# OpenPPL/ppl.llm.serving

Hardware: AMD Instinct MI355X
Metric: decode tokens/sec, LLaMA-7B int8 (W8A16), max-running-batch 1024 (higher is better)
Workload: dtype fp16 activations, int8 weights (W8A16), int8-g8 KV, fp32 accumulate

## Files before the change

ppl.llm.serving_amd/csrc/k_common.h:

```cpp
#pragma once
#include <hip/hip_runtime.h>
#include <hip/hip_fp16.h>
#include <stdint.h>
#include <stdlib.h>

namespace pplhip {

typedef _Float16 h8 __attribute__((ext_vector_type(8)));
typedef _Float16 h4 __attribute__((ext_vector_type(4)));
typedef _Float16 h2 __attribute__((ext_vector_type(2)));
typedef float f4 __attribute__((ext_vector_type(4)));

constexpr int WAVE = 64;

inline int tune_int(const char* name, int dflt) {
#ifdef PPLHIP_TUNING_BUILD
    const char* v = getenv(name);
    return v ? atoi(v) : dflt;
#else
    (void)name;
    return dflt;
#endif
}
inline bool tune_set(const char* name) {
// ... 105 lines not shown
    return w;
}
__device__ __forceinline__ h8 cvt_i4x8_f16(uint32_t w) {
    const uint32_t lo = w & 0x0f0f0f0fu, hi = (w >> 4) & 0x0f0f0f0fu;
    const uint32_t b0 = __builtin_amdgcn_perm(hi, lo, 0x05010400u), b1 = __builtin_amdgcn_perm(hi, lo, 0x07030602u);
    const h2 bias = {(_Float16)1032.0f, (_Float16)1032.0f};
    const h2 a = __builtin_bit_cast(h2, __builtin_amdgcn_perm(0x64646464u, b0, 0x04010400u)) - bias;
    const h2 b = __builtin_bit_cast(h2, __builtin_amdgcn_perm(0x64646464u, b0, 0x04030402u)) - bias;
    const h2 c = __builtin_bit_cast(h2, __builtin_amdgcn_perm(0x64646464u, b1, 0x04010400u)) - bias;
    const h2 d = __builtin_bit_cast(h2, __builtin_amdgcn_perm(0x64646464u, b1, 0x04030402u)) - bias;
    return h8{a[0], a[1], b[0], b[1], c[0], c[1], d[0], d[1]};
}
__device__ __forceinline__ h8 cvt_i4x8_f16(uint32_t w, _Float16 s) { return cvt_i4x8_f16(w) * s; }

#ifndef PPLHIP_KV_NT
#define PPLHIP_KV_NT 1
#endif
typedef uint32_t kv_u32x4 __attribute__((ext_vector_type(4)));
__device__ __forceinline__ uint4 kv_stream_load(const uint4* p) {
#if PPLHIP_KV_NT
    return __builtin_bit_cast(uint4, __builtin_nontemporal_load(reinterpret_cast<const kv_u32x4*>(p)));
#else
    return *p;
#endif
}
__device__ __forceinline__ uint32_t kv_stream_load(const uint32_t* p) {
#if PPLHIP_KV_NT
    return __builtin_nontemporal_load(p);
#else
    return *p;
#endif
}

struct KvStrides {
    int64_t sL, sKV, sH, sN;
};
__host__ __device__ inline KvStrides kv_strides(int layout, int64_t N, int64_t L, int64_t h, int64_t d) {
    KvStrides s;
    switch (layout) {
        case 0: s.sN = L * 2 * h * d; s.sL = 2 * h * d; s.sKV = h * d; s.sH = d; break;
        case 1: s.sL = N * 2 * h * d; s.sN = 2 * h * d; s.sKV = h * d; s.sH = d; break;
        case 2: s.sL = 2 * N * h * d; s.sKV = N * h * d; s.sN = h * d; s.sH = d; break;
        default: s.sL = 2 * h * N * d; s.sKV = h * N * d; s.sH = N * d; s.sN = d; break;
    }
    return s;
}

struct KvAddr {
    void* cache;
    uint16_t* scale;
    int64_t sKV, sH, sN;
    int64_t ssKV, ssH, ssN;
    int32_t mode, page_size;
    int32_t page_shift;
};

__device__ __forceinline__ int64_t kv_slot(const KvAddr& a, const int64_t* __restrict__ cache_indices, int64_t max_pages,
                                           int64_t b, int64_t pos) {
    if (a.mode == 0) return cache_indices[b] + pos;
    if (a.page_shift >= 0) {
        const int64_t pg = pos >> a.page_shift;
        return (cache_indices[b * max_pages + pg] << a.page_shift) + (pos & (int64_t)(a.page_size - 1));
    }
    const int64_t pg = pos / a.page_size;
    return cache_indices[b * max_pages + pg] * a.page_size + (pos - pg * a.page_size);
}
// ... 3 lines not shown
```

ppl.llm.serving_amd/csrc/k_elem.hip:

```cpp
#include <stdlib.h>
#include "kernels.h"

namespace pplhip {

__global__ __launch_bounds__(256) void embedding_kernel(const int64_t* __restrict__ ids, const uint4* __restrict__ table,
                                                        int chunks , uint4* __restrict__ out) {
    const int64_t t = blockIdx.x;
    const int64_t row = ids[t];
    for (int c = threadIdx.x; c < chunks; c += 256) out[t * chunks + c] = table[row * chunks + c];
}

hipError_t launch_embedding(hipStream_t s, const int64_t* token_ids, const uint16_t* table, int64_t T, int hidden,
                            uint16_t* out) {
    if (T == 0) return hipSuccess;
    hipLaunchKernelGGL(embedding_kernel, dim3((unsigned)T), dim3(256), 0, s, token_ids, (const uint4*)table, hidden / 8,
                       (uint4*)out);
    return hipGetLastError();
}

__global__ __launch_bounds__(256) void gather_last_rows_kernel(const int64_t* __restrict__ seq_starts, const uint4* __restrict__ x, int chunks,
                                                               uint4* __restrict__ out) {
    const int64_t r = blockIdx.x, src = seq_starts[r + 1] - 1;
    for (int c = threadIdx.x; c < chunks; c += 256) out[r * chunks + c] = x[src * chunks + c];
}

hipError_t launch_gather_last_rows(hipStream_t s, const uint16_t* x, const int64_t* seq_starts, int64_t B, int hidden, uint16_t* out) {
    if (B == 0) return hipSuccess;
    if (hidden % 8) return hipErrorInvalidValue;
    hipLaunchKernelGGL(gather_last_rows_kernel, dim3((unsigned)B), dim3(256), 0, s, seq_starts, (const uint4*)x, hidden / 8, (uint4*)out);
    return hipGetLastError();
}

template <int MAXC, int NT = 256, bool F8 = false>
__global__ __launch_bounds__(NT) void rmsnorm_kernel(const uint4* x , const uint4* __restrict__ skip,
                                                      const uint4* __restrict__ w, float eps, int chunks, int hidden,
                                                      const int64_t* __restrict__ gather, uint4* __restrict__ out,
                                                      uint4* residual_out, int8_t* __restrict__ qout, float* __restrict__ sx, SplitSlabs sl) {
    __shared__ float red[NT / 64];
    __shared__ float redq[NT / 64];
    const int64_t r = blockIdx.x;
    const int64_t src = gather ? gather[r + 1] - 1 : r;
    float v[MAXC][8];
    float ss = 0.f;
#pragma unroll
    for (int i = 0; i < MAXC; ++i) {
        const int c = threadIdx.x + i * NT;
        if (c < chunks) {
            unpack8(x[src * chunks + c], v[i]);
            if (skip || sl.splits) {
                float sk[8];
                if (sl.splits) slab_load8(sl, src, c * 8, sk);
                else unpack8(skip[src * chunks + c], sk);
#pragma unroll
                for (int j = 0; j < 8; ++j) v[i][j] = round_h(v[i][j] + sk[j]);
                if (residual_out) residual_out[r * chunks + c] = pack8(v[i]);
            } else if (residual_out) {
                residual_out[r * chunks + c] = pack8(v[i]);
            }
#pragma unroll
            for (int j = 0; j < 8; ++j) ss += v[i][j] * v[i][j];
        }
    }
    uint4 wraw[MAXC];
#pragma unroll
    for (int i = 0; i < MAXC; ++i) {
        const int c = threadIdx.x + i * NT;
        wraw[i] = c < chunks ? w[c] : make_uint4(0, 0, 0, 0);
    }
    ss = wave_sum(ss);
    if ((threadIdx.x & 63) == 0) red[threadIdx.x >> 6] = ss;
    __syncthreads();
    ss = red[0] + red[1] + red[2] + red[3];
#pragma unroll
    for (int wv = 4; wv < NT / 64; ++wv) ss += red[wv];
    const float inv = 1.0f / sqrtf(ss / (float)hidden + eps);
    if (!qout) {
#pragma unroll
        for (int i = 0; i < MAXC; ++i) {
            const int c = threadIdx.x + i * NT;
            if (c < chunks) {
                float wf[8], o[8];
                unpack8(wraw[i], wf);
#pragma unroll
                for (int j = 0; j < 8; ++j) o[j] = v[i][j] * inv * wf[j];
                out[r * chunks + c] = pack8(o);
            }
        }
        return;
    }
    float amax = 0.f;
#pragma unroll
    for (int i = 0; i < MAXC; ++i) {
        const int c = threadIdx.x + i * NT;
        if (c < chunks) {
            float wf[8];
            unpack8(wraw[i], wf);
#pragma unroll
            for (int j = 0; j < 8; ++j) {
                v[i][j] = round_h(v[i][j] * inv * wf[j]);
                amax = fmaxf(amax, fabsf(v[i][j]));
            }
        }
    }
#pragma unroll
    for (int o = 32; o > 0; o >>= 1) amax = fmaxf(amax, __shfl_xor(amax, o));
    if ((threadIdx.x & 63) == 0) redq[threadIdx.x >> 6] = amax;
    __syncthreads();
    amax = fmaxf(fmaxf(redq[0], redq[1]), fmaxf(redq[2], redq[3]));
#pragma unroll
    for (int wv = 4; wv < NT / 64; ++wv) amax = fmaxf(amax, redq[wv]);
    if constexpr (F8) {
        const int e = fp8_row_exp(amax);
        if (threadIdx.x == 0) sx[r] = pow2f(e);
#pragma unroll
        for (int i = 0; i < MAXC; ++i) {
            const int c = threadIdx.x + i * NT;
            if (c < chunks) {
                uint32_t lo = 0, hi = 0;
// ... 126 lines not shown
```

ppl.llm.serving_amd/csrc/k_gemm.hip:

```cpp
#include <stdarg.h>
#include <stdio.h>
#include <stdlib.h>

#include <algorithm>

#include <type_traits>
#include "k_gemm_dev.h"

namespace pplhip {

void LinearRoute::add(const char* fmt, ...) {
    if (!buf || cap <= 0 || len >= cap - 1) return;
    if (len > 0) buf[len++] = ' ';
    va_list ap;
    va_start(ap, fmt);
    const int n = vsnprintf(buf + len, (size_t)(cap - len), fmt, ap);
    va_end(ap);
    len = n < 0 ? len : (len + n < cap - 1 ? len + n : cap - 1);
    buf[len] = 0;
}

template <int WQ, int EPI>
__global__ __launch_bounds__(256) void gemm_kernel(const uint16_t* __restrict__ x, const void* __restrict__ wv,
                                                   const uint16_t* __restrict__ scale, int64_t M, int N, int K, int group,
// ... 129 lines not shown
        __syncthreads();
        if (t + 1 < ktiles) {
            store_tile();
            __syncthreads();
        }
    }

#pragma unroll
    for (int i = 0; i < 4; ++i) {
        const int n = n0 + wn * 64 + i * 16 + kq * 4;
        if (n >= N) continue;
        float sc[4] = {1.f, 1.f, 1.f, 1.f};
        if constexpr (WQ == 8) {
            const uint2 s2 = *reinterpret_cast<const uint2*>(scale + n);
            const h4 sh = __builtin_bit_cast(h4, s2);
#pragma unroll
            for (int r = 0; r < 4; ++r) sc[r] = (float)sh[r];
        }
#pragma unroll
        for (int j = 0; j < 4; ++j) {
            const int64_t m = m0 + wm * 64 + j * 16 + l15;
            if (m >= M) continue;
            store4<EPI>(yv, ldy, m, n, acc[i][j][0] * sc[0], acc[i][j][1] * sc[1], acc[i][j][2] * sc[2], acc[i][j][3] * sc[3]);
        }
    }
}

struct DmaKernel { int wq, epi, stages, wl, bm, maxg; };
template <int WQ, int EPI, int G_ST, int WL, int BM = G_BM, int MAXG = W4_MAXG>
__global__ __launch_bounds__(WL == 6 ? 768 : (WL == 5 ? 512 : 256)) void gemm_dma_kernel(const uint16_t* __restrict__ x, const void* __restrict__ wv,
                                                             const uint16_t* __restrict__ scale, int64_t M, int N, int K,
                                                             void* __restrict__ yv, int64_t ldy, int n_tiles, int m_tiles,
                                                             int map_mode, int kt_per_split, float* __restrict__ ws) {
    __shared__ __attribute__((aligned(16))) char smem[gemm_dma_lds_bytes<WQ, G_ST, BM, MAXG>()];
    gemm_dma_body<WQ, EPI, G_ST, WL, BM>(x, wv, scale, M, N, K, yv, ldy, n_tiles, m_tiles, map_mode, kt_per_split, ws, (int)blockIdx.x,
                                     (int)blockIdx.y, (int)gridDim.y, smem);
}

constexpr int S_KS = 2;
constexpr int S_WB = G_BN * G_BK * S_KS;
template <int BM> constexpr int s_xb() { return S_KS * BM * G_BK * 2; }
struct Half128Kernel { int epi, st, bm; };

template <int EPI, int ST, int BM>
__global__ __launch_bounds__(256) void gemm_w8_half128_kernel(const uint16_t* __restrict__ x, const int8_t* __restrict__ w,
                                                              const uint16_t* __restrict__ scale, int64_t M, int N, int K,
                                                              void* __restrict__ yv, int64_t ldy, int n_tiles, int kt_per_split,
                                                              float* __restrict__ ws) {
    constexpr int XB = s_xb<BM>(), NJ = BM / 16;
    constexpr int XP = XB / 1024, WP = S_WB / 1024, PP = (XP + WP) / 4;
    static_assert((XP + WP) % 4 == 0, "every wave issues the same number of pieces");
    extern __shared__ __attribute__((aligned(16))) char smem_h[];
    char* const Xs0 = smem_h;
    char* const Wq0 = smem_h + ST * XB;
    const int nt = blockIdx.x;
    if (nt >= n_tiles) return;
    const int n0 = nt * G_BN;
    const int split_id = blockIdx.y, n_splits = gridDim.y;
    const int tid = threadIdx.x, lane = tid & 63, wave = __builtin_amdgcn_readfirstlane(tid >> 6);
    const int l15 = lane & 15, kq = lane >> 4;
    const int nb = wave * 32;

    const char* psrc[PP];
    uint32_t pdst[PP];
    const uint32_t xbase = lds_addr(Xs0), wbase = lds_addr(Wq0);
#pragma unroll
    for (int j = 0; j < PP; ++j) {
// ... 204 lines not shown
        char* const stg = smem256;
        __syncthreads();
#pragma unroll
        for (int i = 0; i < 2; ++i) {
            const int nl = wn * 32 + i * 16 + kq * 4;
            const int nc = n0 + nl < N ? n0 + nl : 0;
            const h4 sh = __builtin_bit_cast(h4, *reinterpret_cast<const uint2*>(scale + nc));
#pragma unroll
            for (int j = 0; j < 16; ++j) {
                const float v0 = acc[i][j][0] * (float)sh[0], v1 = acc[i][j][1] * (float)sh[1], v2 = acc[i][j][2] * (float)sh[2],
                            v3 = acc[i][j][3] * (float)sh[3];
                char* dst = stg + (j * 16 + l15) * ROWB;
                if constexpr (EPI == EPI_F16) {
                    const h4 o = {to_h(v0), to_h(v1), to_h(v2), to_h(v3)};
                    *reinterpret_cast<uint2*>(dst + nl * 2) = __builtin_bit_cast(uint2, o);
                } else {
                    const float g0 = round_h(v0), u0 = round_h(v1), g1 = round_h(v2), u1 = round_h(v3);
                    const h2 o = {to_h(g0 / (1.0f + __expf(-g0)) * u0), to_h(g1 / (1.0f + __expf(-g1)) * u1)};
                    *reinterpret_cast<uint32_t*>(dst + nl) = __builtin_bit_cast(uint32_t, o);
                }
            }
        }
        __syncthreads();
        uint16_t* const y = reinterpret_cast<uint16_t*>(yv);
        const int nout = EPI == EPI_SWIGLU ? N / 2 : N, c0 = EPI == EPI_SWIGLU ? n0 / 2 : n0;
#pragma unroll 4
        for (int c = tid; c < H_BM * CPR; c += 512) {
            const int row = c / CPR, ch = c - row * CPR;
            const uint4 v = *reinterpret_cast<const uint4*>(stg + row * ROWB + ch * 16);
            const int64_t m = m0 + row;
            const int col = c0 + ch * 8;
            if (m < M) {
                if (col + 8 <= nout) {
                    *reinterpret_cast<uint4*>(y + m * ldy + col) = v;
                } else {
                    const uint16_t* e = reinterpret_cast<const uint16_t*>(&v);
                    for (int k = 0; k < 8; ++k)
                        if (col + k < nout) y[m * ldy + col + k] = e[k];
                }
            }
        }
        return;
    }
#pragma unroll
    for (int i = 0; i < 2; ++i) {
        const int n = n0 + wn * 32 + i * 16 + kq * 4;
        if (n >= N) continue;
        const h4 sh = __builtin_bit_cast(h4, *reinterpret_cast<const uint2*>(scale + n));
#pragma unroll
        for (int j = 0; j < 16; ++j) {
            const int64_t m = m0 + wm * 128 + j * 16 + l15;
            if (m >= M) continue;
            store4<EPI>(yv, ldy, m, n, acc[i][j][0] * (float)sh[0], acc[i][j][1] * (float)sh[1], acc[i][j][2] * (float)sh[2],
                        acc[i][j][3] * (float)sh[3]);
        }
    }
}

template <int WQ, int MT, int EPI, int NW>
__global__ __launch_bounds__(NW * 64) void gemv_kernel(const uint16_t* __restrict__ x, const void* __restrict__ wv,
                                                   const uint16_t* __restrict__ scale, int64_t M, int N, int K, int group,
                                                   void* __restrict__ yv, int64_t ldy) {
    constexpr int KL = WQ == 8 ? 16 : (WQ == 4 ? 32 : 8);
    constexpr int KSTEP = KL * 4;
    constexpr int NKS = KL / 8;
    __shared__ __attribute__((aligned(16))) float red[NW - 1][MT][64][4];
    const int tid = threadIdx.x, lane = tid & 63, wave = tid >> 6;
// ... 373 lines not shown
```

ppl.llm.serving_amd/csrc/k_gemm_dev.h:

```cpp
#pragma once
#include "kernels.h"
#include "k_launch.h"

namespace pplhip {

constexpr int G_BN = 128, G_BM = 128, G_BK = 64;

__device__ __forceinline__ int g_swz(int row, int chunk) { return chunk ^ ((row >> 1) & 7); }

enum { EPI_F16 = 0, EPI_F32 = 1, EPI_SWIGLU = 2 };
template <int EPI>
__device__ __forceinline__ void store4(void* yv, int64_t ldy, int64_t m, int n, float v0, float v1, float v2, float v3) {
    if constexpr (EPI == EPI_F32) {
        *reinterpret_cast<float4*>(reinterpret_cast<float*>(yv) + m * ldy + n) = make_float4(v0, v1, v2, v3);
    } else if constexpr (EPI == EPI_F16) {
        const h4 o = {to_h(v0), to_h(v1), to_h(v2), to_h(v3)};
        *reinterpret_cast<uint2*>(reinterpret_cast<uint16_t*>(yv) + m * ldy + n) = __builtin_bit_cast(uint2, o);
    } else {
        const float g0 = round_h(v0), u0 = round_h(v1), g1 = round_h(v2), u1 = round_h(v3);
        const h2 o = {to_h(g0 / (1.0f + __expf(-g0)) * u0), to_h(g1 / (1.0f + __expf(-g1)) * u1)};
        *reinterpret_cast<uint32_t*>(reinterpret_cast<uint16_t*>(yv) + m * ldy + (n >> 1)) = __builtin_bit_cast(uint32_t, o);
    }
}

template <class F>
inline void dispatch_epi(int epi, F&& f) {
    if (epi == EPI_F32) f(int_c<EPI_F32>{}); else if (epi == EPI_F16) f(int_c<EPI_F16>{}); else f(int_c<EPI_SWIGLU>{});
}
template <class F>
inline void for_each_epi(F&& f) { f(int_c<EPI_F16>{}); f(int_c<EPI_F32>{}); f(int_c<EPI_SWIGLU>{}); }

__device__ __forceinline__ int w_swz(int row) { return (0x1320 >> (((row >> 2) & 3) * 4)) & 3; }

__device__ __forceinline__ h8 cvt_i4x8_f16(uint32_t w, h2 sc) {
    const uint32_t ev = w & 0x0f0f0f0fu, od = (w >> 4) & 0x0f0f0f0fu;
    const h2 bias = {(_Float16)1032.0f, (_Float16)1032.0f};
    const h2 a = (__builtin_bit_cast(h2, __builtin_amdgcn_perm(od, ev, 0x0c040c00u) | 0x64006400u) - bias) * sc;
    const h2 b = (__builtin_bit_cast(h2, __builtin_amdgcn_perm(od, ev, 0x0c050c01u) | 0x64006400u) - bias) * sc;
    const h2 c = (__builtin_bit_cast(h2, __builtin_amdgcn_perm(od, ev, 0x0c060c02u) | 0x64006400u) - bias) * sc;
    const h2 d = (__builtin_bit_cast(h2, __builtin_amdgcn_perm(od, ev, 0x0c070c03u) | 0x64006400u) - bias) * sc;
    return h8{a[0], a[1], b[0], b[1], c[0], c[1], d[0], d[1]};
}

__device__ __forceinline__ void glds16(const void* gsrc, uint32_t lds_wave_base ) {
    uint32_t keep;
    asm volatile("s_mov_b32 %0, m0\n\ts_mov_b32 m0, %2\n\ts_nop 0\n\tglobal_load_lds_dwordx4 %1, off\n\ts_mov_b32 m0, %0"
                 : "=&s"(keep)
                 : "v"(gsrc), "s"(lds_wave_base)
                 : "memory");
}
__device__ __forceinline__ uint32_t lds_addr(const void* p) {
    return (uint32_t)(uintptr_t)(const __attribute__((address_space(3))) char*)p;
}

constexpr int W4_MAXG = 64;

template <int WQ, int G_ST, int BM = G_BM, int MAXG = W4_MAXG>
constexpr int gemm_dma_lds_bytes() {
    constexpr int WB2 = WQ == 8 ? 2 : (WQ == 4 ? 1 : 4);
    return G_ST * (BM * G_BK * 2 + G_BN * G_BK * WB2 / 2) + (WQ == 4 ? MAXG * G_BN * 2 : 0);
}

template <int WQ, int EPI, int G_ST, int WL, int BM = G_BM>
__device__ __forceinline__ void gemm_dma_body(const uint16_t* __restrict__ x, const void* __restrict__ wv,
                                              const uint16_t* __restrict__ scale, int64_t M, int N, int K, void* __restrict__ yv,
                                              int64_t ldy, int n_tiles, int m_tiles, int map_mode, int kt_per_split,
                                              float* __restrict__ ws, int block_id, int split_id, int n_splits, char* smem) {
    constexpr int WB2 = WQ == 8 ? 2 : (WQ == 4 ? 1 : 4);
    constexpr int W_STAGE = G_BN * G_BK * WB2 / 2;
    constexpr int NT = 256;
    static_assert(BM == G_BM || (BM == 64 && WL == 1), "half-height tiles: 4-wave layout only");
    constexpr int X_DMA = BM * G_BK * 2 / (NT * 16);
    constexpr int W_DMA = W_STAGE / (NT * 16);
    uint16_t* const Xs0 = reinterpret_cast<uint16_t*>(smem);
    char* const Wq0 = smem + G_ST * BM * G_BK * 2;
    uint16_t* const Sc = reinterpret_cast<uint16_t*>(smem + G_ST * (BM * G_BK * 2 + W_STAGE));
    const char* w = reinterpret_cast<const char*>(wv);

    const int id = block_id;
    const int xcd = id & 7, slot = id >> 3;
    int nt, mt;
    if ((map_mode & 0xff) == 1) {
        const int mg = m_tiles >> 3;
        mt = xcd + 8 * (slot % mg);
        nt = slot / mg;
    } else {
        const int gm = (map_mode >> 16) & 0xff, gn = (map_mode >> 24) & 0xff;
        if (gm == 0) {
            nt = xcd + 8 * (slot / m_tiles);
            mt = slot % m_tiles;
        } else {
            const int per_super = gn * gm, sm_count = m_tiles / gm;
            const int sup = slot / per_super, within = slot % per_super;
            nt = xcd + 8 * ((sup / sm_count) * gn + within / gm);
            mt = (sup % sm_count) * gm + within % gm;
        }
    }
    if (nt >= n_tiles) return;
    const int n0 = nt * G_BN;
    const int64_t m0 = (int64_t)mt * BM;

    constexpr bool PC = WL == 5 || WL == 6;
    const bool producer = PC && threadIdx.x >= (WL == 6 ? 512 : 256);
    const int tid = PC ? (threadIdx.x & 255) : threadIdx.x, lane = tid & 63, wave = tid >> 6;
    const int kh = WL == 6 ? (int)((threadIdx.x >> 8) & 1) : 0;
    const int l15 = lane & 15, kq = lane >> 4;
    constexpr int NI = WL ? 2 : 4, NJ = WL ? BM / 16 : 4;
    const int wn = WL ? wave : wave >> 1, wm = WL ? 0 : wave & 1;
    const int nb = wn * (NI * 16), mb = wm * (NJ * 16);

    const uint16_t* xsrc[X_DMA];
    const char* wsrc[W_DMA];
#pragma unroll
    for (int j = 0; j < X_DMA; ++j) {
        const int p = j * NT + tid, row = p >> 3, pos = (p & 7) ^ ((row >> 1) & 7);
        const int c = ((pos & 3) << 1) | (pos >> 2);
        int64_t m = m0 + row;
        if (m >= M) m = M - 1;
        xsrc[j] = x + m * K + c * 8;
    }
#pragma unroll
    for (int j = 0; j < W_DMA; ++j) {
        const int p = j * NT + tid;
        if constexpr (WQ == 8) {
            const int row = p >> 2, c = (p & 3) ^ w_swz(row);
            int n = n0 + row;
            if (n >= N) n = N - 1;
            wsrc[j] = w + (int64_t)n * K + c * 16;
        } else if constexpr (WQ == 4) {
            const int row = p >> 1, c = (p & 1) ^ ((row >> 3) & 1);
            int n = n0 + row;
            if (n >= N) n = N - 1;
            wsrc[j] = w + ((int64_t)n * K) / 2 + c * 16;
        } else {
            const int row = p >> 3, pos = (p & 7) ^ ((row >> 1) & 7);
            const int c = ((pos & 3) << 1) | (pos >> 2);
// ... 19 lines not shown

    constexpr int D = G_ST - 1;
    const int kt_all = K / G_BK;
    const int kt0 = split_id * kt_per_split;
    const int ktiles = (kt0 + kt_per_split < kt_all) ? kt_per_split : kt_all - kt0;
    if constexpr (WQ == 4) {
        const int G = K / 128, g0 = kt0 >> 1, ng = (ktiles + 1) >> 1;
        for (int e = tid; e < ng * G_BN; e += NT) {
            const int row = e / ng, g = e - row * ng;
            int n = n0 + row;
            if (n >= N) n = N - 1;
            Sc[g * G_BN + row] = scale[(int64_t)n * G + g0 + g];
        }
        asm volatile("s_waitcnt vmcnt(0)" ::: "memory");
    }
#pragma unroll
    for (int d = 0; d < D; ++d) {
        if (d < ktiles && (!PC || producer)) issue(d, (kt0 + d) * G_BK);
    }
    int st = 0, stn = D;
    h2 gsc[NI];
    if (PC && producer) {
        for (int t = 0; t < ktiles; ++t) {
            const int younger = (ktiles - 1 - t) < (D - 1) ? (ktiles - 1 - t) : (D - 1);
            constexpr int PT = X_DMA + W_DMA;
            if (younger >= 2) asm volatile("s_waitcnt vmcnt(%0)" ::"n"(2 * PT) : "memory");
            else if (younger == 1) asm volatile("s_waitcnt vmcnt(%0)" ::"n"(PT) : "memory");
            else asm volatile("s_waitcnt vmcnt(0)" ::: "memory");
            __syncthreads();
            if (t + D < ktiles) issue(stn, (kt0 + t + D) * G_BK);
            stn = stn == G_ST - 1 ? 0 : stn + 1;
        }
        if constexpr (WL == 6) { __syncthreads(); __syncthreads(); }
        return;
    }
    for (int t = 0; t < ktiles; ++t) {
        const int younger = (ktiles - 1 - t) < (D - 1) ? (ktiles - 1 - t) : (D - 1);
        if constexpr (!PC) {
            constexpr int PT = X_DMA + W_DMA;
            if (map_mode & 0x200) {}
            else if (younger >= 2) asm volatile("s_waitcnt vmcnt(%0)" ::"n"(2 * PT) : "memory");
            else if (younger == 1) asm volatile("s_waitcnt vmcnt(%0)" ::"n"(PT) : "memory");
            else asm volatile("s_waitcnt vmcnt(0)" ::: "memory");
        }
        __syncthreads();
        if constexpr (!PC) if (t + D < ktiles && !(map_mode & 0x100)) issue(stn, (kt0 + t + D) * G_BK);
        const uint16_t* xs = Xs0 + st * (BM * G_BK);
        const char* wq = Wq0 + st * W_STAGE;
        st = st == G_ST - 1 ? 0 : st + 1;
        stn = stn == G_ST - 1 ? 0 : stn + 1;
        uint4 wraw[NI];
        if constexpr (WQ == 8) {
#pragma unroll
            for (int i = 0; i < NI; ++i) {
                const int row = nb + i * 16 + l15;
                wraw[i] = *reinterpret_cast<const uint4*>(&wq[row * G_BK + (kq ^ w_swz(row)) * 16]);
            }
        } else if constexpr (WQ == 4) {
#pragma unroll
            for (int i = 0; i < NI; ++i) {
                const int row = nb + i * 16 + l15;
                const uint2 v = *reinterpret_cast<const uint2*>(&wq[row * 32 + ((kq ^ (((row >> 3) & 1) << 1)) * 8)]);
                wraw[i].x = v.x; wraw[i].y = v.y;
            }
            if ((t & 1) == 0) {
#pragma unroll
// ... 17 lines not shown
                    const int row = nb + i * 16 + l15;
                    a[i] = __builtin_bit_cast(h8, *reinterpret_cast<const uint4*>(&wq[(row * G_BK + g_swz(row, ks * 4 + kq) * 8) * 2]));
                }
            }
#pragma unroll
            for (int j = 0; j < NJ; ++j) {
                const int row = mb + j * 16 + l15;
                bfr[j] = __builtin_bit_cast(h8, *reinterpret_cast<const uint4*>(&xs[row * G_BK + g_swz(row, ks * 4 + kq) * 8]));
            }
#ifdef GEMM_SETPRIO
            __builtin_amdgcn_s_setprio(1);
#endif
#pragma unroll
            for (int i = 0; i < NI; ++i)
#pragma unroll
                for (int j = 0; j < NJ; ++j) acc[i][j] = __builtin_amdgcn_mfma_f32_16x16x32_f16(a[i], bfr[j], acc[i][j], 0, 0, 0);
#ifdef GEMM_SETPRIO
            __builtin_amdgcn_s_setprio(0);
#endif
        }
    }

    if constexpr (WL == 6) {
        float4* red = reinterpret_cast<float4*>(smem);
        __syncthreads();
        if (kh == 1) {
#pragma unroll
            for (int i = 0; i < NI; ++i)
#pragma unroll
                for (int j = 0; j < NJ; ++j)
                    red[((wave * NI + i) * NJ + j) * 64 + lane] = make_float4(acc[i][j][0], acc[i][j][1], acc[i][j][2], acc[i][j][3]);
        }
        __syncthreads();
        if (kh == 1) return;
#pragma unroll
        for (int i = 0; i < NI; ++i)
#pragma unroll
            for (int j = 0; j < NJ; ++j) {
                const float4 o = red[((wave * NI + i) * NJ + j) * 64 + lane];
                acc[i][j][0] += o.x; acc[i][j][1] += o.y; acc[i][j][2] += o.z; acc[i][j][3] += o.w;
            }
    }
    if (n_splits > 1) {
        float* slab = ws + (int64_t)split_id * M * N;
#pragma unroll
        for (int i = 0; i < NI; ++i) {
            const int n = n0 + nb + i * 16 + kq * 4;
            if (n >= N) continue;
#pragma unroll
            for (int j = 0; j < NJ; ++j) {
                const int64_t m = m0 + mb + j * 16 + l15;
                if (m < M) *reinterpret_cast<float4*>(slab + m * N + n) = make_float4(acc[i][j][0], acc[i][j][1], acc[i][j][2], acc[i][j][3]);
            }
        }
        return;
    }
#pragma unroll
    for (int i = 0; i < NI; ++i) {
        const int n = n0 + nb + i * 16 + kq * 4;
        if (n >= N) continue;
        h4 sh = {(_Float16)1.0f, (_Float16)1.0f, (_Float16)1.0f, (_Float16)1.0f};
        if constexpr (WQ == 8) sh = __builtin_bit_cast(h4, *reinterpret_cast<const uint2*>(scale + n));
#pragma unroll
        for (int j = 0; j < NJ; ++j) {
            const int64_t m = m0 + mb + j * 16 + l15;
            if (m >= M) continue;
            store4<EPI>(yv, ldy, m, n, acc[i][j][0] * (float)sh[0], acc[i][j][1] * (float)sh[1], acc[i][j][2] * (float)sh[2],
                        acc[i][j][3] * (float)sh[3]);
        }
    }
}


}
// ... 1 lines not shown
```

ppl.llm.serving_amd/csrc/k_gemm_wide.hip:

```cpp
#include <stdlib.h>
#include "k_gemm_dev.h"

namespace pplhip {

namespace {

constexpr int WD_BM = 128, WD_NP = 4;
constexpr int WD_XB = WD_BM * G_BK * 2;
constexpr int WD_XP = WD_XB / 1024;

template <int EPI, int ST, int NC, int ABL = 0>
__global__ __launch_bounds__((NC + WD_NP) * 64) void gemm_w8_wide_kernel(const uint16_t* __restrict__ x, const int8_t* __restrict__ w,
                                                                  const uint16_t* __restrict__ scale, int64_t M, int N, int K,
                                                                  void* __restrict__ yv, int64_t ldy, int n_tiles, int m_tiles) {
    constexpr int WD_BN = 32 * NC, WD_NC = NC;
    constexpr int WD_WB = WD_BN * G_BK, WD_WP = WD_WB / 1024;
    constexpr int WD_PP = (WD_XP + WD_WP + WD_NP - 1) / WD_NP;
    extern __shared__ __attribute__((aligned(16))) char smem_wd[];
    char* const Xs0 = smem_wd;
    char* const Wq0 = smem_wd + ST * WD_XB;

    const int id = blockIdx.x;
    const int xcd = id & 7, slot = id >> 3;
    const int nt = xcd + 8 * (slot / m_tiles);
    const int mt = slot % m_tiles;
    if (nt >= n_tiles) return;
    const int n0 = nt * WD_BN;
    const int64_t m0 = (int64_t)mt * WD_BM;

    const int tid = threadIdx.x, lane = tid & 63, wave = __builtin_amdgcn_readfirstlane(tid >> 6);
    const int ktiles = K / G_BK;
    constexpr int D = ST - 1;

    if (wave >= WD_NC) {
        const int pw = wave - WD_NC;
        const char* psrc[WD_PP];
        uint32_t pdst[WD_PP];
        const uint32_t xbase = lds_addr(Xs0), wbase = lds_addr(Wq0);
        const int npc = (WD_XP + WD_WP - pw + WD_NP - 1) / WD_NP;
#pragma unroll
        for (int j = 0; j < WD_PP; ++j) {
            const int P = pw + WD_NP * j;
            if (j < WD_XP / WD_NP) {
                const int p = P * 64 + lane, row = p >> 3, pos = (p & 7) ^ ((row >> 1) & 7);
                const int c = ((pos & 3) << 1) | (pos >> 2);
                int64_t m = m0 + row;
                if (m >= M) m = M - 1;
                psrc[j] = reinterpret_cast<const char*>(x + m * K + c * 8);
                pdst[j] = __builtin_amdgcn_readfirstlane(xbase + P * 1024);
            } else {
                const int Pw = (P < WD_XP + WD_WP ? P : WD_XP) - WD_XP;
                const int p = Pw * 64 + lane, row = p >> 2, c = (p & 3) ^ w_swz(row);
                int n = n0 + row;
                if (n >= N) n = N - 1;
                psrc[j] = reinterpret_cast<const char*>(w) + (int64_t)n * K + c * 16;
                pdst[j] = __builtin_amdgcn_readfirstlane(wbase + Pw * 1024);
            }
        }
#define WD_PRODUCE(KT, STG)                                                                                                          \
    do {                                                                                                                             \
        _Pragma("unroll") for (int j = 0; j < WD_PP; ++j)                                                                            \
            if (j < npc)                                                                                                             \
            glds16(psrc[j] + (int64_t)(KT) * (j < WD_XP / WD_NP ? G_BK * 2 : G_BK), pdst[j] + (STG) * (j < WD_XP / WD_NP ? WD_XB : WD_WB)); \
    } while (0)
#pragma unroll
        for (int d = 0; d < D; ++d)
            if (d < ktiles) WD_PRODUCE(d, d);
        int stn = D % ST;
        for (int t = 0; t < ktiles; ++t) {
            const int younger = (ktiles - 1 - t) < (D - 1) ? (ktiles - 1 - t) : (D - 1);
            if (younger >= 2) {
                if (npc == WD_PP) asm volatile("s_waitcnt vmcnt(%0)" ::"n"(2 * WD_PP) : "memory");
                else asm volatile("s_waitcnt vmcnt(%0)" ::"n"(2 * WD_PP - 2) : "memory");
            } else if (younger == 1) {
                if (npc == WD_PP) asm volatile("s_waitcnt vmcnt(%0)" ::"n"(WD_PP) : "memory");
                else asm volatile("s_waitcnt vmcnt(%0)" ::"n"(WD_PP - 1) : "memory");
            } else {
                asm volatile("s_waitcnt vmcnt(0)" ::: "memory");
            }
            if (!(ABL & 8)) __syncthreads();
            if (t + D < ktiles && !(ABL & 1)) WD_PRODUCE(t + D, stn);
            stn = stn == ST - 1 ? 0 : stn + 1;
        }
#undef WD_PRODUCE
        return;
    }

    const int l15 = lane & 15, kq = lane >> 4;
    const int nb = wave * 32;
    f4 acc[2][8];
#pragma unroll
    for (int i = 0; i < 2; ++i)
#pragma unroll
        for (int j = 0; j < 8; ++j) acc[i][j] = f4{0.f, 0.f, 0.f, 0.f};
    int st = 0;
    for (int t = 0; t < ktiles; ++t) {
        if (!(ABL & 8)) __syncthreads();
        const uint16_t* xs = reinterpret_cast<const uint16_t*>(Xs0 + st * WD_XB);
        const char* wq = Wq0 + st * WD_WB;
        st = st == ST - 1 ? 0 : st + 1;
        uint4 wraw[2];
#pragma unroll
        for (int i = 0; i < 2; ++i) {
            const int row = nb + i * 16 + l15;
            wraw[i] = *reinterpret_cast<const uint4*>(&wq[row * G_BK + (kq ^ w_swz(row)) * 16]);
        }
#pragma unroll
        for (int ks = 0; ks < 2; ++ks) {
            h8 a[2], bfr[8];
#pragma unroll
            for (int i = 0; i < 2; ++i) {
                if constexpr (ABL & 2) a[i] = __builtin_bit_cast(h8, make_uint4(wraw[i].x, wraw[i].y, wraw[i].z ^ ks, wraw[i].w));
                else a[i] = cvt_i8x8_f16(ks == 0 ? make_uint2(wraw[i].x, wraw[i].y) : make_uint2(wraw[i].z, wraw[i].w));
            }
#pragma unroll
            for (int j = 0; j < 8; ++j) {
                const int row = j * 16 + l15;
                bfr[j] = __builtin_bit_cast(h8, *reinterpret_cast<const uint4*>(&xs[((ABL & 4) ? 0 : row * G_BK) + g_swz(row, ks * 4 + kq) * 8]));
            }
#pragma unroll
            for (int i = 0; i < 2; ++i)
#pragma unroll
                for (int j = 0; j < 8; ++j) acc[i][j] = __builtin_amdgcn_mfma_f32_16x16x32_f16(a[i], bfr[j], acc[i][j], 0, 0, 0);
        }
    }

#pragma unroll
    for (int i = 0; i < 2; ++i) {
        const int n = n0 + nb + i * 16 + kq * 4;
        if (n >= N) continue;
        const h4 sh = __builtin_bit_cast(h4, *reinterpret_cast<const uint2*>(scale + n));
#pragma unroll
        for (int j = 0; j < 8; ++j) {
            const int64_t m = m0 + j * 16 + l15;
            if (m >= M) continue;
            store4<EPI>(yv, ldy, m, n, acc[i][j][0] * (float)sh[0], acc[i][j][1] * (float)sh[1], acc[i][j][2] * (float)sh[2],
                        acc[i][j][3] * (float)sh[3]);
        }
    }
}

}

int linear_w8_wide_waves(int64_t M, int N) {
    const int64_t m_tiles = (M + WD_BM - 1) / WD_BM;
    const int64_t tiles = (N + 383) / 384 * m_tiles, rounds = (tiles + 255) / 256;
    const double eff = (double)N * (double)M / ((double)rounds * 256.0 * 384.0 * WD_BM);
    return (eff >= 0.85 && (rounds <= 2 || eff >= 0.97)) ? 12 : 0;
}

hipError_t launch_linear_w8_wide(hipStream_t s, const uint16_t* x, const int8_t* w, const uint16_t* scale, int64_t M, int N, int K, void* y,
                                 int64_t ldy, int epi, int nc, LinearRoute* route) {
    if (nc != 12) return hipErrorInvalidValue;
    const int bn = 32 * nc;
    const int n_tiles = (N + bn - 1) / bn, m_tiles = (int)((M + WD_BM - 1) / WD_BM);
    constexpr int ST = 3;
    const size_t lds = (size_t)ST * (WD_XB + bn * G_BK);
    if (route) {
        route->add("kernel=gemm_w8_wide_kernel<%s,%d,%d> splits=1 reduce=none order=plain", epi_name(epi), ST, nc);
// ... 25 lines not shown
```

ppl.llm.serving_amd/csrc/k_rope_kv.hip:

```cpp
#include <stdlib.h>
#include "kernels.h"

namespace pplhip {

template <int QBIT>
__device__ __forceinline__ void store_group8(const KvAddr& kv, int kvsel, int head, int64_t slot, int ch0,
                                             const float* x ) {
    const int64_t base = (int64_t)kvsel * kv.sKV + (int64_t)head * kv.sH + slot * kv.sN + ch0;
    if constexpr (QBIT == 0) {
        *reinterpret_cast<uint4*>(reinterpret_cast<uint16_t*>(kv.cache) + base) = pack8(x);
    } else {
        float mx = 0.f;
#pragma unroll
        for (int i = 0; i < 8; ++i) mx = fmaxf(mx, fabsf(x[i]));
        const _Float16 sh = to_h(mx / 127.0f);
        const float sf = (float)sh;
        const float inv = sf > 0.f ? __fdiv_rn(1.0f, sf) : 0.f;
        uint32_t lo = 0, hi = 0;
#pragma unroll
        for (int i = 0; i < 8; ++i) {
            float q = rintf(__fmul_rn(x[i], inv));
            q = fminf(fmaxf(q, -127.f), 127.f);
            const uint32_t b = (uint32_t)(int)q & 0xffu;
            if (i < 4) lo |= b << (8 * i); else hi |= b << (8 * (i - 4));
        }
        *reinterpret_cast<uint2*>(reinterpret_cast<int8_t*>(kv.cache) + base) = make_uint2(lo, hi);
        const int64_t sbase = (int64_t)kvsel * kv.ssKV + (int64_t)head * kv.ssH + slot * kv.ssN + ch0 / 8;
        kv.scale[sbase] = __builtin_bit_cast(uint16_t, sh);
    }
}

__device__ __forceinline__ void store_fp8_row8(const KvAddr& kv, int kvsel, int head, int64_t slot, int ch0, const float* x ,
                                               int e) {
    const int64_t base = (int64_t)kvsel * kv.sKV + (int64_t)head * kv.sH + slot * kv.sN + ch0;
    const float inv = __builtin_bit_cast(float, (uint32_t)(127 - e) << 23);
    const float lim = e == 8 ? 240.0f : 448.0f;
    uint32_t lo = 0, hi = 0;
#pragma unroll
    for (int i = 0; i < 8; ++i) {
        const float y = __fmul_rn(x[i], inv);
        const uint32_t b = fp8_e4m3_rne(fminf(fmaxf(y, -lim), lim));
        if (i < 4) lo |= b << (8 * i); else hi |= b << (8 * (i - 4));
    }
    *reinterpret_cast<uint2*>(reinterpret_cast<uint8_t*>(kv.cache) + base) = make_uint2(lo, hi);
    if (ch0 == 0) kv.scale[(int64_t)kvsel * kv.ssKV + (int64_t)head * kv.ssH + slot * kv.ssN] = f2h(__builtin_bit_cast(float, (uint32_t)(127 + e) << 23));
}
__device__ __forceinline__ void store_i4_group8(const KvAddr& kv, int kvsel, int head, int64_t slot, int ch0, const float* x , float amax) {
    const float sf = kv_i4_scale(amax);
    const float inv = __fdiv_rn(1.0f, sf);
    const int64_t base = (int64_t)kvsel * kv.sKV + (int64_t)head * kv.sH + slot * kv.sN + ch0 / 2;
    *reinterpret_cast<uint32_t*>(reinterpret_cast<uint8_t*>(kv.cache) + base) = kv_i4_pack8(x, inv);
    if ((ch0 & 31) == 0) kv.scale[(int64_t)kvsel * kv.ssKV + (int64_t)head * kv.ssH + slot * kv.ssN + ch0 / 32] = f2h(sf);
}
__device__ __forceinline__ float group_max(float v, int n) {
    for (int o = 1; o < n; o <<= 1) v = fmaxf(v, __shfl_xor(v, o, 64));
    return v;
}

template <int QBIT>
__global__ __launch_bounds__(256) void rope_kv_write_kernel(uint16_t* __restrict__ qkv, const float* __restrict__ cos_sin,
                                                            KvAddr kv, const int64_t* __restrict__ seq_starts,
                                                            const int64_t* __restrict__ start_pos,
                                                            const int64_t* __restrict__ cache_indices, int64_t max_pages,
                                                            int64_t B, int64_t t0, int H, int Hkv, int D, SplitSlabs sl) {
    const int64_t t = t0 + blockIdx.x;
    int64_t b;
    {
        const int64_t g = t < B ? t : B - 1;
        int64_t lo = 0, hi = B - 1;
        if (seq_starts[g] <= t && t < seq_starts[g + 1]) {
            lo = g;
        } else {
            while (lo < hi) {
                const int64_t mid = (lo + hi + 1) >> 1;
                if (seq_starts[mid] <= t) lo = mid; else hi = mid - 1;
            }
        }
        b = lo;
    }
    const int64_t pos = start_pos[b] + (t - seq_starts[b]);
    const int64_t slot = kv_slot(kv, cache_indices, max_pages, b, pos);
    const int half = D / 2;
    const int bph = half / 8;
    const int n_rope = (H + Hkv) * bph;
    const int n_v = Hkv * (D / 8);
    const int v0 = QBIT == KV_FP8 ? (n_rope + D / 8 - 1) / (D / 8) * (D / 8) : (QBIT == KV_I4G32 ? (n_rope + 3) / 4 * 4 : n_rope);
    uint16_t* row = qkv + t * (int64_t)(H + 2 * Hkv) * D;
    const float* cs = cos_sin + pos * D;
    for (int w = blockIdx.y * 256 + threadIdx.x; w < v0 + n_v; w += 256 * gridDim.y) {
        if (w < n_rope) {
            const int head = w / bph, i0 = (w - head * bph) * 8;
            uint16_t* x = row + (int64_t)head * D;
            float a[8], bb[8], c[8], s[8], ra[8], rb[8];
            if (sl.splits) {
                slab_load8(sl, t - t0, head * D + i0, a);
                slab_load8(sl, t - t0, head * D + i0 + half, bb);
            } else {
                unpack8(*reinterpret_cast<const uint4*>(x + i0), a);
                unpack8(*reinterpret_cast<const uint4*>(x + i0 + half), bb);
            }
            *reinterpret_cast<float4*>(c) = *reinterpret_cast<const float4*>(cs + i0);
            *reinterpret_cast<float4*>(c + 4) = *reinterpret_cast<const float4*>(cs + i0 + 4);
            *reinterpret_cast<float4*>(s) = *reinterpret_cast<const float4*>(cs + half + i0);
            *reinterpret_cast<float4*>(s + 4) = *reinterpret_cast<const float4*>(cs + half + i0 + 4);
#pragma unroll
            for (int i = 0; i < 8; ++i) {
                ra[i] = round_h(__fsub_rn(__fmul_rn(a[i], c[i]), __fmul_rn(bb[i], s[i])));
                rb[i] = round_h(__fadd_rn(__fmul_rn(bb[i], c[i]), __fmul_rn(a[i], s[i])));
            }
            if (head < H) {
                *reinterpret_cast<uint4*>(x + i0) = pack8(ra);
                *reinterpret_cast<uint4*>(x + i0 + half) = pack8(rb);
            } else if constexpr (QBIT == KV_FP8) {
                float mx = 0.f;
#pragma unroll
                for (int i = 0; i < 8; ++i) mx = fmaxf(mx, fmaxf(fabsf(ra[i]), fabsf(rb[i])));
                const int e = fp8_row_exp(group_max(mx, bph));
                store_fp8_row8(kv, 0, head - H, slot, i0, ra, e);
                store_fp8_row8(kv, 0, head - H, slot, i0 + half, rb, e);
            } else if constexpr (QBIT == KV_I4G32) {
                float ma = 0.f, mb = 0.f;
#pragma unroll
                for (int i = 0; i < 8; ++i) { ma = fmaxf(ma, fabsf(ra[i])); mb = fmaxf(mb, fabsf(rb[i])); }
                if (D == 32) ma = mb = group_max(fmaxf(ma, mb), 2);
                else { ma = group_max(ma, 4); mb = group_max(mb, 4); }
                store_i4_group8(kv, 0, head - H, slot, i0, ra, ma);
                store_i4_group8(kv, 0, head - H, slot, i0 + half, rb, mb);
            } else {
                store_group8<QBIT>(kv, 0, head - H, slot, i0, ra);
                store_group8<QBIT>(kv, 0, head - H, slot, i0 + half, rb);
            }
        } else if (w >= v0) {
            const int wv = w - v0;
            const int head = wv / (D / 8), i0 = (wv - head * (D / 8)) * 8;
            float v[8];
            if (sl.splits) slab_load8(sl, t - t0, (H + Hkv + head) * D + i0, v);
            else unpack8(*reinterpret_cast<const uint4*>(row + (int64_t)(H + Hkv + head) * D + i0), v);
            if constexpr (QBIT == KV_FP8) {
                float mx = 0.f;
#pragma unroll
                for (int i = 0; i < 8; ++i) mx = fmaxf(mx, fabsf(v[i]));
                store_fp8_row8(kv, 1, head, slot, i0, v, fp8_row_exp(group_max(mx, D / 8)));
            } else if constexpr (QBIT == KV_I4G32) {
                float mx = 0.f;
#pragma unroll
// ... 44 lines not shown
```

Measured before the change: 23930.

## Stage GEMM epilogue outputs through LDS for coalesced row stores

GEMM epilogues in the wide and producer/consumer DMA kernels now write scaled fp16 or SwiGLU results into an LDS image that reuses the ring buffer. All threads then copy it out as contiguous 16-byte row chunks instead of scattered 4-element fragment stores. The aim is fully coalesced global writes of the output tile, paid for with extra barriers, LDS traffic and a larger LDS allocation for the WL6 variant. Selectable store-cache policies (write-through, nontemporal) are also added for the GEMM, norm and rope/KV stores, but they default to plain stores.

```diff
diff --git a/ppl.llm.serving_amd/csrc/k_common.h b/ppl.llm.serving_amd/csrc/k_common.h
--- a/ppl.llm.serving_amd/csrc/k_common.h
+++ b/ppl.llm.serving_amd/csrc/k_common.h
@@ -161,6 +161,35 @@
 #endif
 }
 
+constexpr int OUT_ST_PLAIN = 0, OUT_ST_WT = 1, OUT_ST_NT = 2;
+template <int POL>
+__device__ __forceinline__ void out_store(uint32_t* p, uint32_t v) {
+    if constexpr (POL == OUT_ST_WT) __hip_atomic_store(p, v, __ATOMIC_RELAXED, __HIP_MEMORY_SCOPE_AGENT);
+    else if constexpr (POL == OUT_ST_NT) __builtin_nontemporal_store(v, p);
+    else *p = v;
+}
+template <int POL>
+__device__ __forceinline__ void out_store(uint2* p, uint2 v) {
+    if constexpr (POL == OUT_ST_WT) __hip_atomic_store(reinterpret_cast<uint64_t*>(p), __builtin_bit_cast(uint64_t, v), __ATOMIC_RELAXED, __HIP_MEMORY_SCOPE_AGENT);
+    else if constexpr (POL == OUT_ST_NT) __builtin_nontemporal_store(__builtin_bit_cast(uint64_t, v), reinterpret_cast<uint64_t*>(p));
+    else *p = v;
+}
+template <int POL>
+__device__ __forceinline__ void out_store(uint4* p, uint4 v) {
+    if constexpr (POL == OUT_ST_WT) asm volatile("global_store_dwordx4 %0, %1, off sc1" ::"v"(p), "v"(__builtin_bit_cast(kv_u32x4, v)) : "memory");
+    else if constexpr (POL == OUT_ST_NT) __builtin_nontemporal_store(__builtin_bit_cast(kv_u32x4, v), reinterpret_cast<kv_u32x4*>(p));
+    else *p = v;
+}
+#ifndef PPLHIP_ST_GEMM
+#define PPLHIP_ST_GEMM 0
+#endif
+#ifndef PPLHIP_ST_NORM
+#define PPLHIP_ST_NORM 0
+#endif
+#ifndef PPLHIP_ST_ROPE
+#define PPLHIP_ST_ROPE 0
+#endif
+
 struct KvStrides {
     int64_t sL, sKV, sH, sN;
 };
diff --git a/ppl.llm.serving_amd/csrc/k_elem.hip b/ppl.llm.serving_amd/csrc/k_elem.hip
--- a/ppl.llm.serving_amd/csrc/k_elem.hip
+++ b/ppl.llm.serving_amd/csrc/k_elem.hip
@@ -53,9 +53,9 @@
                 else unpack8(skip[src * chunks + c], sk);
 #pragma unroll
                 for (int j = 0; j < 8; ++j) v[i][j] = round_h(v[i][j] + sk[j]);
-                if (residual_out) residual_out[r * chunks + c] = pack8(v[i]);
+                if (residual_out) out_store<PPLHIP_ST_NORM>(&residual_out[r * chunks + c], pack8(v[i]));
             } else if (residual_out) {
-                residual_out[r * chunks + c] = pack8(v[i]);
+                out_store<PPLHIP_ST_NORM>(&residual_out[r * chunks + c], pack8(v[i]));
             }
 #pragma unroll
             for (int j = 0; j < 8; ++j) ss += v[i][j] * v[i][j];
@@ -83,7 +83,7 @@
                 unpack8(wraw[i], wf);
 #pragma unroll
                 for (int j = 0; j < 8; ++j) o[j] = v[i][j] * inv * wf[j];
-                out[r * chunks + c] = pack8(o);
+                out_store<PPLHIP_ST_NORM>(&out[r * chunks + c], pack8(o));
             }
         }
         return;
diff --git a/ppl.llm.serving_amd/csrc/k_gemm.hip b/ppl.llm.serving_amd/csrc/k_gemm.hip
--- a/ppl.llm.serving_amd/csrc/k_gemm.hip
+++ b/ppl.llm.serving_amd/csrc/k_gemm.hip
@@ -185,7 +185,7 @@
                                                              const uint16_t* __restrict__ scale, int64_t M, int N, int K,
                                                              void* __restrict__ yv, int64_t ldy, int n_tiles, int m_tiles,
                                                              int map_mode, int kt_per_split, float* __restrict__ ws) {
-    __shared__ __attribute__((aligned(16))) char smem[gemm_dma_lds_bytes<WQ, G_ST, BM, MAXG>()];
+    __shared__ __attribute__((aligned(16))) char smem[gemm_dma_lds_bytes<WQ, G_ST, BM, MAXG, WL>()];
     gemm_dma_body<WQ, EPI, G_ST, WL, BM>(x, wv, scale, M, N, K, yv, ldy, n_tiles, m_tiles, map_mode, kt_per_split, ws, (int)blockIdx.x,
                                      (int)blockIdx.y, (int)gridDim.y, smem);
 }
@@ -456,7 +456,7 @@
             const int col = c0 + ch * 8;
             if (m < M) {
                 if (col + 8 <= nout) {
-                    *reinterpret_cast<uint4*>(y + m * ldy + col) = v;
+                    out_store<PPLHIP_ST_GEMM>(reinterpret_cast<uint4*>(y + m * ldy + col), v);
                 } else {
                     const uint16_t* e = reinterpret_cast<const uint16_t*>(&v);
                     for (int k = 0; k < 8; ++k)
diff --git a/ppl.llm.serving_amd/csrc/k_gemm_dev.h b/ppl.llm.serving_amd/csrc/k_gemm_dev.h
--- a/ppl.llm.serving_amd/csrc/k_gemm_dev.h
+++ b/ppl.llm.serving_amd/csrc/k_gemm_dev.h
@@ -23,6 +23,51 @@
     }
 }
 
+#ifndef PPLHIP_GEMM_STAGE_WIDE
+#define PPLHIP_GEMM_STAGE_WIDE 1
+#endif
+#ifndef PPLHIP_GEMM_STAGE_DMA
+#define PPLHIP_GEMM_STAGE_DMA 1
+#endif
+template <int EPI, int BN>
+constexpr int out_stage_row_bytes() { return (EPI == EPI_SWIGLU ? BN / 2 : BN) * 2 + 16; }
+template <int EPI, int BN>
+constexpr int out_stage_bytes() { return 128 * out_stage_row_bytes<EPI, BN>(); }
+template <int EPI>
+__device__ __forceinline__ bool out_stage_ok(const void* yv, int64_t ldy, int N) {
+    if constexpr (EPI == EPI_F32) return false;
+    return ldy % 8 == 0 && (reinterpret_cast<uintptr_t>(yv) & 15) == 0 && (EPI != EPI_SWIGLU || N % 16 == 0);
+}
+template <int EPI>
+__device__ __forceinline__ void out_stage_put4(char* row, int nl, float v0, float v1, float v2, float v3) {
+    static_assert(EPI != EPI_F32, "fp32 outputs keep the direct epilogue");
+    if constexpr (EPI == EPI_F16) {
+        const h4 o = {to_h(v0), to_h(v1), to_h(v2), to_h(v3)};
+        *reinterpret_cast<uint2*>(row + nl * 2) = __builtin_bit_cast(uint2, o);
+    } else {
+        const float g0 = round_h(v0), u0 = round_h(v1), g1 = round_h(v2), u1 = round_h(v3);
+        const h2 o = {to_h(g0 / (1.0f + __expf(-g0)) * u0), to_h(g1 / (1.0f + __expf(-g1)) * u1)};
+        *reinterpret_cast<uint32_t*>(row + nl) = __builtin_bit_cast(uint32_t, o);
+    }
+}
+template <int EPI, int BN, int NTHR>
+__device__ __forceinline__ void out_stage_copy(const char* stg, int t, void* yv, int64_t ldy, int64_t m0, int64_t M, int n0, int N) {
+    constexpr int ROWB = out_stage_row_bytes<EPI, BN>(), CPR = (ROWB - 16) / 16;
+    uint16_t* const y = reinterpret_cast<uint16_t*>(yv);
+    const int nout = EPI == EPI_SWIGLU ? N / 2 : N, c0 = EPI == EPI_SWIGLU ? n0 / 2 : n0;
+    static_assert(128 * CPR % NTHR == 0, "whole passes of the copying threads");
+#pragma unroll
+    for (int it = 0; it < 128 * CPR / NTHR; ++it) {
+        const int c = t + it * NTHR, row = c / CPR, ch = c - row * CPR;
+        const uint4 v = *reinterpret_cast<const uint4*>(stg + row * ROWB + ch * 16);
+        const int64_t m = m0 + row;
+        const int col = c0 + ch * 8;
+        if (m >= M || col >= nout) continue;
+        if (col + 8 <= nout) out_store<PPLHIP_ST_GEMM>(reinterpret_cast<uint4*>(y + m * ldy + col), v);
+        else out_store<PPLHIP_ST_GEMM>(reinterpret_cast<uint2*>(y + m * ldy + col), make_uint2(v.x, v.y));
+    }
+}
+
 template <class F>
 inline void dispatch_epi(int epi, F&& f) {
     if (epi == EPI_F32) f(int_c<EPI_F32>{}); else if (epi == EPI_F16) f(int_c<EPI_F16>{}); else f(int_c<EPI_SWIGLU>{});
@@ -55,10 +100,13 @@
 
 constexpr int W4_MAXG = 64;
 
-template <int WQ, int G_ST, int BM = G_BM, int MAXG = W4_MAXG>
+constexpr int DMA_WL6_RED_BYTES = 4 * 2 * (G_BM / 16) * 64 * 16;
+template <int WQ, int G_ST, int BM = G_BM, int MAXG = W4_MAXG, int WL = 1>
 constexpr int gemm_dma_lds_bytes() {
     constexpr int WB2 = WQ == 8 ? 2 : (WQ == 4 ? 1 : 4);
-    return G_ST * (BM * G_BK * 2 + G_BN * G_BK * WB2 / 2) + (WQ == 4 ? MAXG * G_BN * 2 : 0);
+    constexpr int ring = G_ST * (BM * G_BK * 2 + G_BN * G_BK * WB2 / 2) + (WQ == 4 ? MAXG * G_BN * 2 : 0);
+    constexpr int wl6 = DMA_WL6_RED_BYTES + out_stage_bytes<EPI_F16, G_BN>();
+    return WL == 6 && ring < wl6 ? wl6 : ring;
 }
 
 template <int WQ, int EPI, int G_ST, int WL, int BM = G_BM>
@@ -102,6 +150,10 @@
 
     constexpr bool PC = WL == 5 || WL == 6;
     const bool producer = PC && threadIdx.x >= (WL == 6 ? 512 : 256);
+    constexpr bool STG = PPLHIP_GEMM_STAGE_DMA && PC && BM == G_BM && WQ != 4 && EPI != EPI_F32;
+    constexpr int STG_OFF = WL == 6 ? DMA_WL6_RED_BYTES : 0;
+    static_assert(!STG || STG_OFF + out_stage_bytes<EPI, G_BN>() <= gemm_dma_lds_bytes<WQ, G_ST, BM, W4_MAXG, WL>(), "the output image fits the ring");
+    const bool staged = STG && n_splits == 1 && out_stage_ok<EPI>(yv, ldy, N);
     const int tid = PC ? (threadIdx.x & 255) : threadIdx.x, lane = tid & 63, wave = tid >> 6;
     const int kh = WL == 6 ? (int)((threadIdx.x >> 8) & 1) : 0;
     const int l15 = lane & 15, kq = lane >> 4;
@@ -187,6 +239,12 @@
             stn = stn == G_ST - 1 ? 0 : stn + 1;
         }
         if constexpr (WL == 6) { __syncthreads(); __syncthreads(); }
+        if constexpr (STG) {
+            if (staged) {
+                if constexpr (WL == 5) __syncthreads();
+                __syncthreads();
+            }
+        }
         return;
     }
     for (int t = 0; t < ktiles; ++t) {
@@ -270,7 +328,15 @@
                     red[((wave * NI + i) * NJ + j) * 64 + lane] = make_float4(acc[i][j][0], acc[i][j][1], acc[i][j][2], acc[i][j][3]);
         }
         __syncthreads();
-        if (kh == 1) return;
+        if (kh == 1) {
+            if constexpr (STG) {
+                if (staged) {
+                    __syncthreads();
+                    out_stage_copy<EPI, G_BN, 512>(smem + STG_OFF, (int)threadIdx.x, yv, ldy, m0, M, n0, N);
+                }
+            }
+            return;
+        }
 #pragma unroll
         for (int i = 0; i < NI; ++i)
 #pragma unroll
@@ -278,6 +344,26 @@
                 const float4 o = red[((wave * NI + i) * NJ + j) * 64 + lane];
                 acc[i][j][0] += o.x; acc[i][j][1] += o.y; acc[i][j][2] += o.z; acc[i][j][3] += o.w;
             }
+    }
+    if constexpr (STG) {
+        if (staged) {
+            constexpr int ROWB = out_stage_row_bytes<EPI, G_BN>();
+            char* const stg = smem + STG_OFF;
+            if constexpr (WL == 5) __syncthreads();
+#pragma unroll
+            for (int i = 0; i < NI; ++i) {
+                const int nl = nb + i * 16 + kq * 4;
+                h4 sh = {(_Float16)1.0f, (_Float16)1.0f, (_Float16)1.0f, (_Float16)1.0f};
+                if constexpr (WQ == 8) sh = __builtin_bit_cast(h4, *reinterpret_cast<const uint2*>(scale + (n0 + nl < N ? n0 + nl : 0)));
+#pragma unroll
+                for (int j = 0; j < NJ; ++j)
+                    out_stage_put4<EPI>(stg + (j * 16 + l15) * ROWB, nl, acc[i][j][0] * (float)sh[0], acc[i][j][1] * (float)sh[1],
+                                        acc[i][j][2] * (float)sh[2], acc[i][j][3] * (float)sh[3]);
+            }
+            __syncthreads();
+            out_stage_copy<EPI, G_BN, WL == 6 ? 512 : 256>(stg, (int)threadIdx.x, yv, ldy, m0, M, n0, N);
+            return;
+        }
     }
     if (n_splits > 1) {
         float* slab = ws + (int64_t)split_id * M * N;
diff --git a/ppl.llm.serving_amd/csrc/k_gemm_wide.hip b/ppl.llm.serving_amd/csrc/k_gemm_wide.hip
--- a/ppl.llm.serving_amd/csrc/k_gemm_wide.hip
+++ b/ppl.llm.serving_amd/csrc/k_gemm_wide.hip
@@ -31,6 +31,8 @@
     const int tid = threadIdx.x, lane = tid & 63, wave = __builtin_amdgcn_readfirstlane(tid >> 6);
     const int ktiles = K / G_BK;
     constexpr int D = ST - 1;
+    const bool staged = PPLHIP_GEMM_STAGE_WIDE && out_stage_ok<EPI>(yv, ldy, N);
+    static_assert(EPI == EPI_F32 || out_stage_bytes<EPI, WD_BN>() <= ST * (WD_XB + WD_WB), "the output image fits the ring");
 
     if (wave >= WD_NC) {
         const int pw = wave - WD_NC;
@@ -83,6 +85,7 @@
             stn = stn == ST - 1 ? 0 : stn + 1;
         }
 #undef WD_PRODUCE
+        if (staged) { __syncthreads(); __syncthreads(); }
         return;
     }
 
@@ -125,6 +128,25 @@
         }
     }
 
+    if constexpr (EPI != EPI_F32) {
+        if (staged) {
+            constexpr int ROWB = out_stage_row_bytes<EPI, WD_BN>();
+            __syncthreads();
+#pragma unroll
+            for (int i = 0; i < 2; ++i) {
+                const int nl = nb + i * 16 + kq * 4;
+                const int nc = n0 + nl < N ? n0 + nl : 0;
+                const h4 sh = __builtin_bit_cast(h4, *reinterpret_cast<const uint2*>(scale + nc));
+#pragma unroll
+                for (int j = 0; j < 8; ++j)
+                    out_stage_put4<EPI>(smem_wd + (j * 16 + l15) * ROWB, nl, acc[i][j][0] * (float)sh[0], acc[i][j][1] * (float)sh[1],
+                                        acc[i][j][2] * (float)sh[2], acc[i][j][3] * (float)sh[3]);
+            }
+            __syncthreads();
+            out_stage_copy<EPI, WD_BN, WD_NC * 64>(smem_wd, tid, yv, ldy, m0, M, n0, N);
+            return;
+        }
+    }
 #pragma unroll
     for (int i = 0; i < 2; ++i) {
         const int n = n0 + nb + i * 16 + kq * 4;
diff --git a/ppl.llm.serving_amd/csrc/k_rope_kv.hip b/ppl.llm.serving_amd/csrc/k_rope_kv.hip
--- a/ppl.llm.serving_amd/csrc/k_rope_kv.hip
+++ b/ppl.llm.serving_amd/csrc/k_rope_kv.hip
@@ -8,7 +8,7 @@
                                              const float* x ) {
     const int64_t base = (int64_t)kvsel * kv.sKV + (int64_t)head * kv.sH + slot * kv.sN + ch0;
     if constexpr (QBIT == 0) {
-        *reinterpret_cast<uint4*>(reinterpret_cast<uint16_t*>(kv.cache) + base) = pack8(x);
+        out_store<PPLHIP_ST_ROPE>(reinterpret_cast<uint4*>(reinterpret_cast<uint16_t*>(kv.cache) + base), pack8(x));
     } else {
         float mx = 0.f;
 #pragma unroll
@@ -24,7 +24,7 @@
             const uint32_t b = (uint32_t)(int)q & 0xffu;
             if (i < 4) lo |= b << (8 * i); else hi |= b << (8 * (i - 4));
         }
-        *reinterpret_cast<uint2*>(reinterpret_cast<int8_t*>(kv.cache) + base) = make_uint2(lo, hi);
+        out_store<PPLHIP_ST_ROPE>(reinterpret_cast<uint2*>(reinterpret_cast<int8_t*>(kv.cache) + base), make_uint2(lo, hi));
         const int64_t sbase = (int64_t)kvsel * kv.ssKV + (int64_t)head * kv.ssH + slot * kv.ssN + ch0 / 8;
         kv.scale[sbase] = __builtin_bit_cast(uint16_t, sh);
     }
@@ -42,14 +42,14 @@
         const uint32_t b = fp8_e4m3_rne(fminf(fmaxf(y, -lim), lim));
         if (i < 4) lo |= b << (8 * i); else hi |= b << (8 * (i - 4));
     }
-    *reinterpret_cast<uint2*>(reinterpret_cast<uint8_t*>(kv.cache) + base) = make_uint2(lo, hi);
+    out_store<PPLHIP_ST_ROPE>(reinterpret_cast<uint2*>(reinterpret_cast<uint8_t*>(kv.cache) + base), make_uint2(lo, hi));
     if (ch0 == 0) kv.scale[(int64_t)kvsel * kv.ssKV + (int64_t)head * kv.ssH + slot * kv.ssN] = f2h(__builtin_bit_cast(float, (uint32_t)(127 + e) << 23));
 }
 __device__ __forceinline__ void store_i4_group8(const KvAddr& kv, int kvsel, int head, int64_t slot, int ch0, const float* x , float amax) {
     const float sf = kv_i4_scale(amax);
     const float inv = __fdiv_rn(1.0f, sf);
     const int64_t base = (int64_t)kvsel * kv.sKV + (int64_t)head * kv.sH + slot * kv.sN + ch0 / 2;
-    *reinterpret_cast<uint32_t*>(reinterpret_cast<uint8_t*>(kv.cache) + base) = kv_i4_pack8(x, inv);
+    out_store<PPLHIP_ST_ROPE>(reinterpret_cast<uint32_t*>(reinterpret_cast<uint8_t*>(kv.cache) + base), kv_i4_pack8(x, inv));
     if ((ch0 & 31) == 0) kv.scale[(int64_t)kvsel * kv.ssKV + (int64_t)head * kv.ssH + slot * kv.ssN + ch0 / 32] = f2h(sf);
 }
 __device__ __forceinline__ float group_max(float v, int n) {
@@ -109,8 +109,8 @@
                 rb[i] = round_h(__fadd_rn(__fmul_rn(bb[i], c[i]), __fmul_rn(a[i], s[i])));
             }
             if (head < H) {
-                *reinterpret_cast<uint4*>(x + i0) = pack8(ra);
-                *reinterpret_cast<uint4*>(x + i0 + half) = pack8(rb);
+                out_store<PPLHIP_ST_ROPE>(reinterpret_cast<uint4*>(x + i0), pack8(ra));
+                out_store<PPLHIP_ST_ROPE>(reinterpret_cast<uint4*>(x + i0 + half), pack8(rb));
             } else if constexpr (QBIT == KV_FP8) {
                 float mx = 0.f;
 #pragma unroll
```

Result: no change. 23990, median of 6 (+0.3%).
